# indygreg/python-zstandard

Hardware: NVIDIA H100
Metric: uncompressed GB/s (compress+decompress) (higher is better)
Workload: dtype u8

## Files before the change

python_zstandard_b200/csrc/zb_decode.cu:

```cuda
#include "zb_common.cuh"
#ifdef ZB_SIMT_EMULATION
#define ZB_DYN_SMEM(name) u8* const name = simt_dyn_smem;
#else
#define ZB_DYN_SMEM(name) extern __shared__ __align__(16) u8 name[];
#endif

#ifdef ZB_DEBUG_BLOCKS
#include <cstdio>
#endif

__constant__ u8 c_LL_bits[36] = {0,0,0,0,0,0,0,0,0,0,0,0,0,0,0,0,1,1,1,1,2,2,3,3,4,6,7,8,9,10,11,12,13,14,15,16};
__constant__ u8 c_ML_bits[53] = {0,0,0,0,0,0,0,0,0,0,0,0,0,0,0,0,0,0,0,0,0,0,0,0,0,0,0,0,0,0,0,0,
                                 1,1,1,1,2,2,3,3,4,4,5,7,8,9,10,11,12,13,14,15,16};
__constant__ u32 c_LL_base[36] = {0,1,2,3,4,5,6,7,8,9,10,11,12,13,14,15,16,18,20,22,24,28,32,40,48,64,
                                  0x80,0x100,0x200,0x400,0x800,0x1000,0x2000,0x4000,0x8000,0x10000};
__constant__ u32 c_ML_base[53] = {3,4,5,6,7,8,9,10,11,12,13,14,15,16,17,18,19,20,21,22,23,24,25,26,27,28,29,30,31,32,33,34,
                                  35,37,39,41,43,47,51,59,67,83,99,0x83,0x103,0x203,0x403,0x803,0x1003,0x2003,0x4003,0x8003,0x10003};
__constant__ short c_LL_defnorm[36] = {4,3,2,2,2,2,2,2,2,2,2,2,2,1,1,1,2,2,2,2,2,2,2,2,2,3,2,1,1,1,1,1,-1,-1,-1,-1};
__constant__ short c_ML_defnorm[53] = {1,4,3,2,2,2,2,2,2,1,1,1,1,1,1,1,1,1,1,1,1,1,1,1,1,1,1,1,1,1,1,1,
                                       1,1,1,1,1,1,1,1,1,1,1,1,1,1,-1,-1,-1,-1,-1,-1,-1};
__constant__ short c_OF_defnorm[29] = {1,1,1,1,1,1,2,2,2,1,1,1,1,1,1,1,1,1,1,1,1,1,1,1,-1,-1,-1,-1,-1};

enum { K_LL = 0, K_OF = 1, K_ML = 2 };

// ... 329 lines not shown
        int count; int low = (int)r.peek((u32)(nbits - 1));
        if (low < mx) { count = low; r.skip((u32)(nbits - 1)); }
        else { count = (int)r.peek((u32)nbits); if (count >= threshold) count -= mx; r.skip((u32)nbits); }
        count--;
        remaining -= count < 0 ? -count : count;
        norm[sym++] = (short)count;
        prev0 = !count;
        if (remaining < threshold) {
            if (remaining <= 1) break;
            nbits = zb_hibit((u32)remaining) + 1; threshold = 1 << (nbits - 1);
        }
        if (sym >= max_sv1) break;
    }
    if (remaining != 1 || sym > max_sv1 || r.bp > 8 * n) return 0;
    max_sym = sym - 1;
    return (r.bp + 7) >> 3;
}

__device__ __forceinline__ u32 zb_code_add_bits(u32 sym, int kind)
{
    return kind == K_LL ? c_LL_bits[sym] : (kind == K_ML ? c_ML_bits[sym] : sym);
}

template <typename Cell = ZbFseCell>
__device__ static void zb_build_fse(Cell* t, short* norm, u32 max_sym, u32 log, int kind)
{
    u32 const size = 1u << log, mask = size - 1, step = (size >> 1) + (size >> 3) + 3;
    u32 high = size - 1;
    for (u32 s = 0; s <= max_sym; s++) if (norm[s] == -1) { t[high--] = (Cell)s; norm[s] = 0x4001; }
    u32 pos = 0;
    for (u32 s = 0; s <= max_sym; s++) {
        int const c = norm[s];
        if (c & 0x4000) { norm[s] = 1; continue; }
        for (int i = 0; i < c; i++) { t[pos] = (Cell)s; do pos = (pos + step) & mask; while (pos > high); }
    }
    for (u32 u = 0; u < size; u++) {
        u32 const s = t[u], x = (u32)(u16)norm[s]; norm[s] = (short)(x + 1);
        u32 const nb = log - (u32)zb_hibit(x);
        if constexpr (sizeof(Cell) == 4) t[u] = ZB_CELL((x << nb) - size, nb, zb_code_add_bits(s, kind), s);
        else t[u] = ZB_CELL16(s, x);
    }
}

__global__ void zb_build_default_tables()
{
    if (threadIdx.x == 0 && blockIdx.x == 0) {
        short norm[64];
        for (int i = 0; i < 36; i++) norm[i] = c_LL_defnorm[i];
        zb_build_fse(g_defLL, norm, 35, 6, K_LL);
        for (int i = 0; i < 29; i++) norm[i] = c_OF_defnorm[i];
        zb_build_fse(g_defOF, norm, 28, 5, K_OF);
        for (int i = 0; i < 53; i++) norm[i] = c_ML_defnorm[i];
        zb_build_fse(g_defML, norm, 52, 6, K_ML);
    }
}

struct ZbTab { u32 off; u32 log; };

// ... 1054 lines not shown
                          u32* __restrict__ first_error)
{
    u32 f = blockIdx.x * blockDim.x + threadIdx.x;
    if (f >= n_frames) return;
    ZbSegment s; s.offset = place[f].dst_off; s.length = out_sizes[f];
    out_segs[f] = s;
    if (status[f] != ZB_OK) atomicMin(first_error, f);
}

__global__ void zb_chain_shift(ZbFramePlace* __restrict__ place, u32 n_entries, u64 carry)
{
    u32 const i = blockIdx.x * blockDim.x + threadIdx.x;
    if (i < n_entries) place[i].dst_off += carry;
}

__global__ void zb_digest_dict(const u8* __restrict__ dict, u32 n, ZbDictDigest* __restrict__ out)
{
    if (threadIdx.x || blockIdx.x) return;
    out->status = ZB_OK; out->has_entropy = 0; out->dict_id = 0; out->content_off = 0;
    if (n < 8 || zb_rd32(dict) != ZB_MAGIC_DICT) return;
    out->dict_id = zb_rd32(dict + 4);
    const u8* p = dict + 8; const u8* const end = dict + n;
    {
        __align__(16) u8 ws[256]; u32 rank[13], log, nsym;
#ifdef __CUDA_ARCH__
        __shared__ __align__(16) u8 ring[64];
#else
        u8* const ring = nullptr;
#endif
        u32 const used = zb_huf_weights(ws, p, (u32)(end - p), log, nsym, rank, ring);
        if (!used) { out->status = ZB_E_DICT_CORRUPTED; return; }
        zb_huf_fill(out->huf, ws, log, nsym, rank, 0, 0);
        out->huf_log = log; p += used;
        u32 mxs = 0;
        for (u32 i = 0; i < 256; i++) {
            u32 const wt = i < nsym ? (ws[i >> 1] >> ((i & 1) * 4)) & 15 : 0;
            out->c_huf_nb[i] = wt ? (u8)(log + 1 - wt) : 0; if (wt) mxs = i;
        }
        out->c_huf_max = mxs;
    }
    short norm[64]; u32 mx, log, used;
    mx = 31; used = zb_read_ncount(norm, mx, log, p, (u32)(end - p));
    if (!used || log > 8) { out->status = ZB_E_DICT_CORRUPTED; return; }
    for (u32 i = 0; i < 32; i++) out->c_norm_of[i] = i <= mx ? norm[i] : 0; out->c_max_of = mx;
    zb_build_fse(out->of, norm, mx, log, K_OF); out->of_log = log; p += used;
    mx = 52; used = zb_read_ncount(norm, mx, log, p, (u32)(end - p));
    if (!used || log > 9) { out->status = ZB_E_DICT_CORRUPTED; return; }
// ... 187 lines not shown
```

python_zstandard_b200/csrc/zb_entropy.cuh:

```cuda
#pragma once

#define ZB_ENT_WS_BYTES   256
#define ZB_ENT_DEF_LL     512
#define ZB_ENT_DEF_OF     (ZB_ENT_DEF_LL + 2 * 64)
#define ZB_ENT_DEF_ML     (ZB_ENT_DEF_OF + 2 * 32)
#define ZB_ENT_HEAD_BYTES (ZB_ENT_DEF_ML + 2 * 64)
#define ZB_ENT_POOL_BYTES(W) ((((227 * 1024 - ZB_ENT_HEAD_BYTES) / (W))) & ~15)
#define ZB_ENT_SMEM(W)    ((W) * ZB_ENT_POOL_BYTES(W) + ZB_ENT_HEAD_BYTES)

enum : u32 { ZB_SRC_NONE = 0, ZB_SRC_PREDEF = 1, ZB_SRC_RLE = 2, ZB_SRC_NCOUNT = 3, ZB_SRC_DICT = 4 };
struct ZbTabSrc { u32 kind; u32 sym; const u8* p; u32 n; };

enum : u32 { ZB_BD_FIRST = 1, ZB_BD_FSE_VALID = 2, ZB_BD_SKIP = 4 };
struct ZbBlkDesc {
    u64 hdr_off;
    u64 seq_off, lit_off;
    u32 span;
    u32 frame;
    u32 flags;
    u32 block_max;
    ZbTabSrc dHuf, dLL, dOF, dML;
};
struct ZbBlkExit { u32 rep[3]; u32 err; };

__device__ __forceinline__ u32 zb_warp_incl_scan(u32 v, u32 lane)
{
    #pragma unroll
    for (int d = 1; d < 32; d <<= 1) { u32 y = __shfl_up_sync(0xFFFFFFFFu, v, d); if (lane >= (u32)d) v += y; }
    return v;
}

__device__ static u32 zb_huf_weights(u8* ws, const u8* s, u32 n, u32& out_log, u32& out_nsym, u32* rank, ZB_RING_ARG(ring))
{
    u8* const wn = ws;
    u16* const wt = (u16*)(ws + 128);
    u32 nsym, hdr;
    if (n == 0) return 0;
    #pragma unroll
    for (int i = 0; i < 13; i++) rank[i] = 0;
    for (int i = 0; i < 32; i++) ((u32*)wn)[i] = 0;
    u32 total = 0;
    auto put = [&](u32 i, u32 w) { wn[i >> 1] |= (u8)(w << ((i & 1) * 4)); };
    if (s[0] >= 128) {
        nsym = (u32)s[0] - 127; hdr = (nsym + 1) / 2;
        if (hdr + 1 > n) return 0;
        for (u32 i = 0; i < nsym; i++) {
            u32 b = s[1 + i / 2], w = (i & 1) ? (b & 15) : (b >> 4);
            if (w > 12) return 0;
            put(i, w); rank[w]++; total += (1u << w) >> 1;
        }
    } else {
        hdr = s[0];
        if (hdr + 1 > n) return 0;
        short norm[16]; u32 max_sym = 255, log;
        {
            short nn[256];
            u32 used = zb_read_ncount(nn, max_sym, log, s + 1, hdr);
            if (used == 0 || log > 6) return 0;
            for (u32 i = 16; i <= max_sym; i++) if (nn[i]) return 0;
            if (max_sym > 15) max_sym = 15;
            for (u32 i = 0; i <= max_sym; i++) norm[i] = nn[i];
            u32 const size = 1u << log, mask = size - 1, step = (size >> 1) + (size >> 3) + 3;
            u32 high = size - 1, pos = 0;
            u8 next[16];
            for (u32 sy = 0; sy <= max_sym; sy++) {
                if (norm[sy] == -1) { wt[high--] = (u16)sy; next[sy] = 1; } else next[sy] = (u8)norm[sy];
            }
            for (u32 sy = 0; sy <= max_sym; sy++) {
                int const c = norm[sy];
                for (int i = 0; i < c; i++) { wt[pos] = (u16)sy; do pos = (pos + step) & mask; while (pos > high); }
            }
            for (u32 u = 0; u < size; u++) {
                u32 const sy = wt[u], x = next[sy]++;
                u32 const nb = log - (u32)zb_hibit(x);
                wt[u] = (u16)(sy | (nb << 4) | (((x << nb) - size) << 8));
            }
            ZbBitR<4> b;
            if (!b.init(s + 1 + used, hdr - used, ring)) return 0;
            u32 s1 = b.read(log), s2 = b.read(log); b.refill();
            if (b.left() < 0) return 0;
            nsym = 0;
            for (;;) {
                if (nsym + 2 > 255) return 0;
                { u32 c = wt[s1], w = c & 15; if (w > 12) return 0; put(nsym, w); rank[w]++; total += (1u << w) >> 1; nsym++;
                  s1 = (c >> 8) + b.read((c >> 4) & 15); b.refill(); }
                if (b.left() < 0) { u32 w = wt[s2] & 15; if (w > 12) return 0; put(nsym, w); rank[w]++; total += (1u << w) >> 1; nsym++; break; }
                if (nsym + 2 > 255) return 0;
                { u32 c = wt[s2], w = c & 15; if (w > 12) return 0; put(nsym, w); rank[w]++; total += (1u << w) >> 1; nsym++;
                  s2 = (c >> 8) + b.read((c >> 4) & 15); b.refill(); }
                if (b.left() < 0) { u32 w = wt[s1] & 15; if (w > 12) return 0; put(nsym, w); rank[w]++; total += (1u << w) >> 1; nsym++; break; }
            }
        }
    }
    if (total == 0) return 0;
    u32 const log = (u32)zb_hibit(total) + 1;
    if (log > 12) return 0;
    u32 const rest = (1u << log) - total, hb = (u32)zb_hibit(rest);
    if ((1u << hb) != rest) return 0;
    put(nsym, hb + 1); rank[hb + 1]++; nsym++;
    if (rank[1] < 2 || (rank[1] & 1)) return 0;
    out_log = log; out_nsym = nsym;
    return hdr + 1;
}

#define ZB_HUF_COARSE 8u
struct ZbHufTab { const u16* cells; u32 log, shift, T, base; };
__device__ __forceinline__ void zb_huf_shape(u32 log, const u32* rank, u32& shift, u32& T, u32& base, u32& bytes)
{
    shift = log > ZB_HUF_COARSE ? log - ZB_HUF_COARSE : 0u;
    T = 0; for (u32 wt = 1; wt <= shift; wt++) T += rank[wt] << (wt - 1);
    base = (T + 3u) & ~3u;
    bytes = 2u * (base + (1u << (log - shift)));
}
__device__ __forceinline__ ZbHufTab zb_huf_full(const u16* cells, u32 log) { ZbHufTab t; t.cells = cells; t.log = log; t.shift = 0; t.T = 0; t.base = 0; return t; }
#define ZB_HCELL(t, v) ((t).cells[(v) < (t).T ? (v) : (t).base + ((v) >> (t).shift)])

__device__ static void zb_huf_fill(u16* cells, const u8* ws, u32 log, u32 nsym, const u32* rank, u32 shift, u32 base)
{
    u32 start[13]; { u32 p = 0; for (u32 wt = 1; wt <= 12; wt++) { start[wt] = p; p += wt <= log ? (rank[wt] << (wt - 1)) : 0; } }
    for (u32 i = 0; i < nsym; i++) {
        u32 const wt = (ws[i >> 1] >> ((i & 1) * 4)) & 15; if (!wt) continue;
        u32 len = 1u << (wt - 1), p = start[wt]; start[wt] = p + len;
        if (wt > shift) { len >>= shift; p = base + (p >> shift); }
        u32 const cell = i | ((log + 1 - wt) << 8);
        if (len >= 4) { u64 const v = cell * 0x0001000100010001ull; u64* q = (u64*)(cells + p); for (u32 k = 0; k < len / 4; k++) q[k] = v; }
        else if (len == 2) *(u32*)(cells + p) = cell * 0x00010001u;
        else cells[p] = (u16)cell;
    }
}

__device__ static bool zb_huf_stream2(u8* out, u32 n_out, const u8* s, u32 n, ZbHufTab const t, u8* ring)
{
    ZbBitR<4> b;
    if (!b.init(s, n, ring)) return false;
    u32 const log = t.log;
    u32 i = 0;
    while (i < n_out && ((uintptr_t)(out + i) & 3)) { u32 v = b.peek(log); u32 c = ZB_HCELL(t, v); out[i++] = (u8)c; b.skip(c >> 8); b.refill(); }
    for (; i + 4 <= n_out; i += 4) {
        u32 v0 = b.peek(log); u32 c0 = ZB_HCELL(t, v0); b.skip(c0 >> 8);
        u32 v1 = b.peek(log); u32 c1 = ZB_HCELL(t, v1); b.skip(c1 >> 8); b.refill();
        u32 v2 = b.peek(log); u32 c2 = ZB_HCELL(t, v2); b.skip(c2 >> 8);
        u32 v3 = b.peek(log); u32 c3 = ZB_HCELL(t, v3); b.skip(c3 >> 8); b.refill();
        *(u32*)(out + i) = (c0 & 255) | ((c1 & 255) << 8) | ((c2 & 255) << 16) | (c3 << 24);
    }
    for (; i < n_out; i++) { u32 v = b.peek(log); u32 c = ZB_HCELL(t, v); out[i] = (u8)c; b.skip(c >> 8); b.refill(); }
    return b.left() == 0;
}

struct ZbHufLane { ZbBitR<4> b; u8* out; u32 left; };

__device__ __forceinline__ void zb_huf_one(ZbHufLane& h, ZbHufTab const& t)
{
// ... 66 lines not shown
{
    zb_cta_for(1u << log, [&](u32 i) { u32 const c = src[i]; ((u16*)dst)[i] = ZB_CELL16(ZB_CELL_SYM(c), (ZB_CELL_NEXT(c) + (1u << log)) >> ZB_CELL_NB(c)); });
}

template <int W>
__device__ __forceinline__ u32 zb_ent_head(u8* smem, ZbDictDev const& dict)
{
    u32* const lutLL = (u32*)smem; u32* const lutML = lutLL + 36;
    zb_cta_for(36, [&](u32 i) { lutLL[i] = c_LL_base[i] | ((u32)c_LL_bits[i] << 24); });
    zb_cta_for(53, [&](u32 i) { lutML[i] = c_ML_base[i] | ((u32)c_ML_bits[i] << 24); });
    zb_cta_cells16(smem + ZB_ENT_DEF_LL, g_defLL, 6);
    zb_cta_cells16(smem + ZB_ENT_DEF_OF, g_defOF, 5);
    zb_cta_cells16(smem + ZB_ENT_DEF_ML, g_defML, 6);
    u32 head = ZB_ENT_HEAD_BYTES;
    if (dict.has_entropy) {
        zb_cta_cells16(smem + head, dict.ll, dict.ll_log); head += 2u << dict.ll_log;
        zb_cta_cells16(smem + head, dict.of, dict.of_log); head += 2u << dict.of_log;
        zb_cta_cells16(smem + head, dict.ml, dict.ml_log); head += 2u << dict.ml_log;
    }
    __syncthreads();
    return ((ZB_ENT_SMEM(W) - head) / W) & ~15u;
}

template <bool SYMREP>
__device__ __forceinline__ u32 zb_seq_block(const u8* smem, u8* q, u8* ws, ZbDictDev const& dict,
                                            ZbTabSrc const& dLL, ZbTabSrc const& dOF, ZbTabSrc const& dML,
                                            u32 msLL, u32 msOF, u32 msML, u32 logLL, u32 logOF, u32 logML,
                                            const u8* ip, const u8* bend, u32 nseq, ZbSeq* sq, u32 n_lit, u64 room, u64 hist,
                                            u32& rep0, u32& rep1, u32& rep2, u32& lit_used, u32& produced)
{
    const u32* const lutLL = (const u32*)smem; const u32* const lutML = lutLL + 36;
    short* const normLL = (short*)ws; short* const normOF = normLL + 36; short* const normML = normOF + 32;
    u32 const dct_ll = ZB_ENT_HEAD_BYTES, dct_of = dct_ll + (2u << dict.ll_log), dct_ml = dct_of + (2u << dict.of_log);
    ZbTab tLL, tOF, tML;
    auto setup = [&](const ZbTabSrc& d, short* norm, u32 ms, u32 lg, int kind, u32 dct, u32 dlog, u32 def, u32 deflog, ZbTab& t) {
        if (d.kind == ZB_SRC_NCOUNT) { zb_build_fse((u16*)q, norm, ms, lg, kind); t.off = (u32)(q - smem); t.log = lg; q += 2u << lg; }
        else if (d.kind == ZB_SRC_RLE) { *(u16*)q = ZB_CELL16(d.sym, 1u); t.off = (u32)(q - smem); t.log = 0; q += 2; }
        else if (d.kind == ZB_SRC_DICT) { t.off = dct; t.log = dlog; }
        else { t.off = def; t.log = deflog; }
    };
    setup(dLL, normLL, msLL, logLL, K_LL, dct_ll, dict.ll_log, ZB_ENT_DEF_LL, 6, tLL);
    setup(dOF, normOF, msOF, logOF, K_OF, dct_of, dict.of_log, ZB_ENT_DEF_OF, 5, tOF);
    setup(dML, normML, msML, logML, K_ML, dct_ml, dict.ml_log, ZB_ENT_DEF_ML, 6, tML);

    ZbBitR<8> b;
    if (!b.init(ip, (u32)(bend - ip), ws)) return ZB_E_CORRUPTION;
    u32 sLL = b.read(tLL.log); u32 sOF = b.read(tOF.log); b.refill(); u32 sML = b.read(tML.log);
    const u8* const TL = smem + tLL.off; const u8* const TO = smem + tOF.off; const u8* const TM = smem + tML.off;
    u32 const kL = 31 - tLL.log, kO = 31 - tOF.log, kM = 31 - tML.log;
    u32 err = ZB_OK;
    for (u32 i = 0; i < nseq; i++) {
        u32 const cl = *(const u16*)(TL + 2 * sLL), co = *(const u16*)(TO + 2 * sOF), cm = *(const u16*)(TM + 2 * sML);
        b.refill();
        u32 const llc = cl & 63, ofc = co & 63, xl = cl >> 6, xo = co >> 6, xm = cm >> 6;
        u32 const nl = __clz(xl) - kL, nm = __clz(xm) - kM, no = __clz(xo) - kO;
        u32 const eL = lutLL[llc], eM = lutML[cm & 63];
        u32 const llb = eL >> 24, ab = (eM >> 24) + llb;
        u32 const sb = i + 1 < nseq ? nl + nm + no : 0;
        bool const slow = (int)(ofc + ab + sb) > b.avail;
        u32 const ob = b.read(ofc);
        u32 ll = eL & 0xFFFFFFu, ml = eM & 0xFFFFFFu, off;
        if (ofc > 1) {
            off = (1u << ofc) - 3 + ob;
            if (SYMREP && (off & 0x80000000u)) { err = ZB_E_CORRUPTION; break; }
            rep2 = rep1; rep1 = rep0; rep0 = off;
        } else {
// ... 13 lines not shown
        if (slow) b.refill();
        {
            u32 const both = b.read(ab);
            ml += both >> llb; ll += both & ((1u << llb) - 1);
        }
        if (slow) b.refill();
        {
            u32 const v = b.read(sb);
            sLL = (xl << nl) - (1u << tLL.log) + (v >> (nm + no));
            sML = (xm << nm) - (1u << tML.log) + ((v >> no) & ((1u << nm) - 1));
            sOF = (xo << no) - (1u << tOF.log) + (v & ((1u << no) - 1));
        }
        sq[i] = make_uint4(lit_used, produced, ml, off);
        if ((u64)produced + ll + ml > room) { err = ZB_E_DSTSIZE_TOO_SMALL; break; }
        if (ll > n_lit - lit_used) { err = ZB_E_CORRUPTION; break; }
        lit_used += ll; produced += ll;
        if ((u64)off > hist + produced) { err = ZB_E_CORRUPTION; break; }
        produced += ml;
    }
    if (!err && b.left() != 0) err = ZB_E_CORRUPTION;
    return err;
}

#ifdef ZB_PHASE_TIMERS
__device__ unsigned long long g_zb_ent_phase[8];
#define ZB_EMARK(k) do { if (lane == 0) { long long const t_ = clock64(); atomicAdd(&g_zb_ent_phase[k], (unsigned long long)(t_ - t_ph)); t_ph = t_; } } while (0)
#elif defined(ZB_DEBUG_BLOCKS)
#define ZB_EMARK(k) do { if (err && !(t_ph & 1)) { printf("[emark %d] lane %u err %u\n", k, lane, err); t_ph |= 1; } } while (0)
#else
#define ZB_EMARK(k) do { (void)t_ph; } while (0)
#endif

template <int ZB_ENT_WARPS>
__global__ void __launch_bounds__(ZB_ENT_WARPS * 32)
zb_entropy_decode(const u8* __restrict__ src, const ZbSegment* __restrict__ segs, u32 n_frames,
                  const ZbFramePlace* __restrict__ place, const u64* __restrict__ dst_sizes,
                  ZbBlock* __restrict__ blocks, ZbSeq* __restrict__ seqs, u8* __restrict__ lits,
                  u32* __restrict__ work_counter, ZbDictDev dict, u32* status, u64* __restrict__ out_sizes,
                  u32* __restrict__ ck_expect, u32 take)
{
    ZB_DYN_SMEM(zb_smem);
    u32 const lane = threadIdx.x & 31, warp = threadIdx.x >> 5;
    u32 const pool_bytes = zb_ent_head<ZB_ENT_WARPS>(zb_smem, dict);
    u8* const pool = zb_smem + ZB_ENT_SMEM(ZB_ENT_WARPS) - (ZB_ENT_WARPS - warp) * pool_bytes;
    u8* const ws = pool + lane * ZB_ENT_WS_BYTES;
    u8* const tabs = pool + 32 * ZB_ENT_WS_BYTES;
    u32 const TAB_BYTES = pool_bytes - 32 * ZB_ENT_WS_BYTES;

    for (;;) {
        u32 base = 0;
        if (lane == 0) base = atomicAdd(work_counter, take);
        base = __shfl_sync(0xFFFFFFFFu, base, 0);
        if (base >= n_frames) return;
        u32 const f = base + lane;
        bool done = lane >= take || !(f < n_frames) || status[f] != ZB_OK;

        const u8* s = src; u64 n = 0; ZbHdr h; ZbFramePlace pl; u32 err = ZB_OK;
        u64 cap = 0, out_pos = 0, blk_i = 0, seq_i = 0, lit_i = 0, pos = 0; u32 block_max = 0;
        u32 rep0 = 1, rep1 = 4, rep2 = 8;
        ZbTabSrc dHuf = {ZB_SRC_NONE, 0, nullptr, 0}, dLL = dHuf, dOF = dHuf, dML = dHuf;
        bool fse_valid = false;
        if (!done) {
            s = src + segs[f].offset; n = segs[f].length;
            zb_skip_skippable(s, n);
            zb_parse_header(s, n, h);
            pl = place[f]; cap = pl.dst_cap; blk_i = pl.blk_off; seq_i = pl.seq_off; lit_i = pl.lit_off; pos = h.hdr_size;
            block_max = h.window < ZB_BLOCK_MAX ? (u32)h.window : ZB_BLOCK_MAX;
            if (dict.has_entropy) {
                dHuf.kind = dLL.kind = dOF.kind = dML.kind = ZB_SRC_DICT; fse_valid = true;
                rep0 = dict.rep[0]; rep1 = dict.rep[1]; rep2 = dict.rep[2];
// ... 17 lines not shown
                    if (type == 3) { err = ZB_E_CORRUPTION; break; }
                    if (type == ZB_BLK_RLE) {
                        if (pos + 1 > n) { err = ZB_E_SRCSIZE_WRONG; break; }
                        if (bsize > block_max) { err = ZB_E_CORRUPTION; break; }
                        if (bsize > cap - out_pos) { err = ZB_E_DSTSIZE_TOO_SMALL; break; }
                        B.src_pos = (u64)(s + pos - src); B.regen = bsize; B.lit_byte = s[pos]; pos += 1;
                    } else if (type == ZB_BLK_RAW) {
                        if (pos + bsize > n) { err = ZB_E_SRCSIZE_WRONG; break; }
                        if (bsize > block_max) { err = ZB_E_CORRUPTION; break; }
                        if (bsize > cap - out_pos) { err = ZB_E_DSTSIZE_TOO_SMALL; break; }
                        B.src_pos = (u64)(s + pos - src); B.regen = bsize; pos += bsize;
                    } else {
                        if (pos + bsize > n || bsize > block_max) { err = ZB_E_SRCSIZE_WRONG; break; }
                        bs = s + pos; bend = bs + bsize;
                        err = zb_parse_lit_header(bs, bsize, L);
                        if (err) break;
                        if (L.regen > block_max) { err = ZB_E_CORRUPTION; break; }
                        B.n_lit = L.regen; comp = true;
                    }
                } while (0);
                if (err) { done = true; comp = false; }
            }
            ZB_EMARK(1);
            bool wantH = false; u32 hlog = 0, hns = 0; u32 rank[13]; const u8* hp = nullptr; u32 hleft = 0;
            if (comp) {
                do {
                    if (L.type == 0) {
                        if (L.hdr + L.regen > bsize) { err = ZB_E_CORRUPTION; break; }
                        B.lit_kind = ZB_LIT_RAW; B.src_pos = (u64)(bs + L.hdr - src); ip = bs + L.hdr + L.regen;
                    } else if (L.type == 1) {
                        if (L.hdr + 1 > bsize) { err = ZB_E_CORRUPTION; break; }
                        B.lit_kind = ZB_LIT_RLE; B.lit_byte = bs[L.hdr]; ip = bs + L.hdr + 1;
                    } else {
                        if (L.type == 3 && dHuf.kind == ZB_SRC_NONE) { err = ZB_E_DICT_CORRUPTED; break; }
                        if (!L.single && L.regen < 6) { err = ZB_E_LITERALS_HEADER_WRONG; break; }
                        if (L.csize + L.hdr > bsize || L.regen == 0) { err = ZB_E_CORRUPTION; break; }
                        hp = bs + L.hdr; hleft = L.csize;
                        if (L.type == 2) { dHuf.kind = ZB_SRC_NCOUNT; dHuf.p = hp; dHuf.n = hleft; }
                        if (dHuf.kind == ZB_SRC_NCOUNT) {
                            u32 const used = zb_huf_weights(ws, dHuf.p, dHuf.n, hlog, hns, rank, tabs + lane * 64);
                            if (used == 0 || (L.type == 2 && used >= hleft)) { err = ZB_E_CORRUPTION; break; }
                            if (L.type == 2) { hp += used; hleft -= used; dHuf.n = used; }
                            wantH = true;
                        }
                        B.lit_kind = ZB_LIT_SCRATCH; B.src_pos = lit_i; ip = bs + L.hdr + L.csize;
                    }
                } while (0);
                if (err) { done = true; comp = false; wantH = false; }
            }
            if (comp && B.lit_kind == ZB_LIT_SCRATCH && dHuf.kind == ZB_SRC_DICT) {
                if (!zb_huf_block(lits + lit_i, L.regen, hp, hleft, L.single, zb_huf_full(dict.huf, dict.huf_log), ws)) { err = ZB_E_CORRUPTION; done = true; comp = false; }
            }
            ZB_EMARK(2);
            {
                bool pending = wantH;
                u32 hshift = 0, hT = 0, hbase = 0, hbytes = 0;
                if (wantH) zb_huf_shape(hlog, rank, hshift, hT, hbase, hbytes);
                while (__any_sync(0xFFFFFFFFu, pending)) {
                    u32 const need = pending ? hbytes : 0;
                    u32 const incl = zb_warp_incl_scan((need + 15) & ~15u, lane);
                    if (pending && incl <= TAB_BYTES) {
                        u16* cells = (u16*)(tabs + incl - ((need + 15) & ~15u));
                        zb_huf_fill(cells, ws, hlog, hns, rank, hshift, hbase);
                        ZbHufTab t; t.cells = cells; t.log = hlog; t.shift = hshift; t.T = hT; t.base = hbase;
                        if (!zb_huf_block(lits + lit_i, L.regen, hp, hleft, L.single, t, ws)) { err = ZB_E_CORRUPTION; done = true; comp = false; }
                        pending = false;
                    }
                    __syncwarp();
                }
            }
            ZB_EMARK(3);
            if (comp && B.lit_kind == ZB_LIT_SCRATCH) lit_i += (L.regen + 15) & ~15u;
            u32 nseq = 0, logLL = 0, logOF = 0, logML = 0, msLL = 0, msOF = 0, msML = 0, needS = 0;
            short* const normLL = (short*)ws; short* const normOF = normLL + 36; short* const normML = normOF + 32;
            if (comp) {
                do {
                    if (ip >= bend) { err = ZB_E_SRCSIZE_WRONG; break; }
                    nseq = *ip++;
                    if (nseq > 0x7F) {
                        if (nseq == 0xFF) { if (ip + 2 > bend) { err = ZB_E_SRCSIZE_WRONG; break; } nseq = zb_rd16(ip) + 0x7F00; ip += 2; }
                        else { if (ip >= bend) { err = ZB_E_SRCSIZE_WRONG; break; } nseq = ((nseq - 0x80) << 8) + *ip++; }
                    }
                    B.n_seq = nseq;
                    if (nseq == 0) { if (ip != bend) err = ZB_E_CORRUPTION; break; }
                    if (ip + 1 > bend) { err = ZB_E_SRCSIZE_WRONG; break; }
                    u32 const modes = *ip++;
                    if (modes & 3) { err = ZB_E_CORRUPTION; break; }
                    u32 nd; int r;
                    r = zb_seq_desc(dLL, modes >> 6, 35, 9, ip, (u32)(bend - ip), fse_valid, normLL, logLL, msLL, nd);
                    if (r < 0) { err = ZB_E_CORRUPTION; break; } ip += r; needS += nd;
                    r = zb_seq_desc(dOF, (modes >> 4) & 3, 31, 8, ip, (u32)(bend - ip), fse_valid, normOF, logOF, msOF, nd);
                    if (r < 0) { err = ZB_E_CORRUPTION; break; } ip += r; needS += nd;
                    r = zb_seq_desc(dML, (modes >> 2) & 3, 52, 9, ip, (u32)(bend - ip), fse_valid, normML, logML, msML, nd);
                    if (r < 0) { err = ZB_E_CORRUPTION; break; } ip += r; needS += nd;
                    fse_valid = true;
                } while (0);
                if (err) { done = true; comp = false; nseq = 0; }
            }
            ZB_EMARK(4);
            u32 lit_used = 0, produced = 0;
            {
                bool pending = comp && nseq > 0;
                while (__any_sync(0xFFFFFFFFu, pending)) {
                    u32 const need = pending ? ((needS + 15) & ~15u) : 0;
                    u32 const incl = zb_warp_incl_scan(need, lane);
                    if (pending && incl <= TAB_BYTES) {
                        err = zb_seq_block<false>(zb_smem, tabs + incl - need, ws, dict, dLL, dOF, dML, msLL, msOF, msML, logLL, logOF, logML,
                                                   ip, bend, nseq, seqs + seq_i, L.regen, cap - out_pos, out_pos + hist_extra,
                                                   rep0, rep1, rep2, lit_used, produced);
                        if (err) { done = true; comp = false; }
                        pending = false;
                    }
                    __syncwarp();
                }
            }
            ZB_EMARK(5);
            if (!done) {
                if (comp) {
                    seqs[seq_i + nseq] = make_uint4(lit_used, produced, 0, 0);
                    seq_i += nseq + 1;
                    u32 const tail = L.regen - lit_used;
                    if ((u64)produced + tail > cap - out_pos) err = ZB_E_DSTSIZE_TOO_SMALL;
                    B.regen = produced + tail;
                    if (!err && B.regen > block_max) err = ZB_E_CORRUPTION;
                    pos += bsize;
                }
                if (!err) {
                    blocks[blk_i++] = B;
                    out_pos += B.regen;
                    if (last) {
                        if (h.content_size != ZB_CONTENT_UNKNOWN && out_pos != h.content_size) err = ZB_E_CORRUPTION;
                        else if (h.checksum && pos + 4 > n) err = ZB_E_CHECKSUM_WRONG;
// ... 65 lines not shown
                    if (type == 3) { err = ZB_E_CORRUPTION; break; }
                    if (type == ZB_BLK_RLE) {
                        if (pos + 1 > n) { err = ZB_E_SRCSIZE_WRONG; break; }
                        if (bsize > block_max) { err = ZB_E_CORRUPTION; break; }
                        if (bsize > cap - out_pos) { err = ZB_E_DSTSIZE_TOO_SMALL; break; }
                        B.src_pos = (u64)(s + pos - src); B.regen = bsize; B.lit_byte = s[pos]; pos += 1;
                    } else if (type == ZB_BLK_RAW) {
                        if (pos + bsize > n) { err = ZB_E_SRCSIZE_WRONG; break; }
                        if (bsize > block_max) { err = ZB_E_CORRUPTION; break; }
                        if (bsize > cap - out_pos) { err = ZB_E_DSTSIZE_TOO_SMALL; break; }
                        B.src_pos = (u64)(s + pos - src); B.regen = bsize; pos += bsize;
                    } else {
                        if (pos + bsize > n || bsize > block_max) { err = ZB_E_SRCSIZE_WRONG; break; }
                        bs = s + pos; bend = bs + bsize;
                        err = zb_parse_lit_header(bs, bsize, L);
                        if (err) break;
                        if (L.regen > block_max) { err = ZB_E_CORRUPTION; break; }
                        B.n_lit = L.regen; comp = true;
                    }
                } while (0);
                if (err) { done = true; comp = false; }
            }
            ZB_EMARK(1);
            bool wantH = false; u32 hlog = 0, hns = 0; u32 rank[13]; const u8* hp = nullptr; u32 hleft = 0;
            if (comp) {
                do {
                    if (L.type == 0) {
                        if (L.hdr + L.regen > bsize) { err = ZB_E_CORRUPTION; break; }
                        B.lit_kind = ZB_LIT_RAW; B.src_pos = (u64)(bs + L.hdr - src); ip = bs + L.hdr + L.regen;
                    } else if (L.type == 1) {
                        if (L.hdr + 1 > bsize) { err = ZB_E_CORRUPTION; break; }
                        B.lit_kind = ZB_LIT_RLE; B.lit_byte = bs[L.hdr]; ip = bs + L.hdr + 1;
                    } else {
                        if (L.type == 3 && dHuf.kind == ZB_SRC_NONE) { err = ZB_E_DICT_CORRUPTED; break; }
                        if (!L.single && L.regen < 6) { err = ZB_E_LITERALS_HEADER_WRONG; break; }
                        if (L.csize + L.hdr > bsize || L.regen == 0) { err = ZB_E_CORRUPTION; break; }
                        hp = bs + L.hdr; hleft = L.csize;
                        if (L.type == 2) { dHuf.kind = ZB_SRC_NCOUNT; dHuf.p = hp; dHuf.n = hleft; }
                        if (dHuf.kind == ZB_SRC_NCOUNT) {
                            u32 const used = zb_huf_weights(ws, dHuf.p, dHuf.n, hlog, hns, rank, tabs + lane * 64);
                            if (used == 0 || (L.type == 2 && used >= hleft)) { err = ZB_E_CORRUPTION; break; }
                            if (L.type == 2) { hp += used; hleft -= used; dHuf.n = used; }
                            wantH = true;
                        }
                        B.lit_kind = ZB_LIT_SCRATCH; B.src_pos = lit_i; ip = bs + L.hdr + L.csize;
                    }
                } while (0);
                if (err) { done = true; comp = false; wantH = false; }
            }
            if (comp && B.lit_kind == ZB_LIT_SCRATCH && dHuf.kind == ZB_SRC_DICT) {
                if (!zb_huf_block(lits + lit_i, L.regen, hp, hleft, L.single, zb_huf_full(dict.huf, dict.huf_log), ws)) { err = ZB_E_CORRUPTION; done = true; comp = false; }
            }
            ZB_EMARK(2);
            {
                bool pending = wantH;
                u32 hshift = 0, hT = 0, hbase = 0, hbytes = 0;
                if (wantH) zb_huf_shape(hlog, rank, hshift, hT, hbase, hbytes);
                while (__any_sync(0xFFFFFFFFu, pending)) {
                    u32 const need = pending ? hbytes : 0;
                    u32 const incl = zb_warp_incl_scan((need + 15) & ~15u, lane);
                    if (pending && incl <= TAB_BYTES) {
                        u16* cells = (u16*)(tabs + incl - ((need + 15) & ~15u));
                        zb_huf_fill(cells, ws, hlog, hns, rank, hshift, hbase);
                        ZbHufTab t; t.cells = cells; t.log = hlog; t.shift = hshift; t.T = hT; t.base = hbase;
                        if (!zb_huf_block(lits + lit_i, L.regen, hp, hleft, L.single, t, ws)) { err = ZB_E_CORRUPTION; done = true; comp = false; }
                        pending = false;
                    }
                    __syncwarp();
                }
            }
            ZB_EMARK(3);
            if (comp && B.lit_kind == ZB_LIT_SCRATCH) lit_i += (L.regen + 15) & ~15u;
            u32 nseq = 0, logLL = 0, logOF = 0, logML = 0, msLL = 0, msOF = 0, msML = 0, needS = 0;
            short* const normLL = (short*)ws; short* const normOF = normLL + 36; short* const normML = normOF + 32;
            if (comp) {
                do {
                    if (ip >= bend) { err = ZB_E_SRCSIZE_WRONG; break; }
                    nseq = *ip++;
                    if (nseq > 0x7F) {
                        if (nseq == 0xFF) { if (ip + 2 > bend) { err = ZB_E_SRCSIZE_WRONG; break; } nseq = zb_rd16(ip) + 0x7F00; ip += 2; }
                        else { if (ip >= bend) { err = ZB_E_SRCSIZE_WRONG; break; } nseq = ((nseq - 0x80) << 8) + *ip++; }
                    }
                    B.n_seq = nseq;
                    if (nseq == 0) { if (ip != bend) err = ZB_E_CORRUPTION; break; }
                    if (ip + 1 > bend) { err = ZB_E_SRCSIZE_WRONG; break; }
                    u32 const modes = *ip++;
                    if (modes & 3) { err = ZB_E_CORRUPTION; break; }
                    u32 nd; int r;
                    r = zb_seq_desc(dLL, modes >> 6, 35, 9, ip, (u32)(bend - ip), fse_valid, normLL, logLL, msLL, nd);
                    if (r < 0) { err = ZB_E_CORRUPTION; break; } ip += r; needS += nd;
                    r = zb_seq_desc(dOF, (modes >> 4) & 3, 31, 8, ip, (u32)(bend - ip), fse_valid, normOF, logOF, msOF, nd);
                    if (r < 0) { err = ZB_E_CORRUPTION; break; } ip += r; needS += nd;
                    r = zb_seq_desc(dML, (modes >> 2) & 3, 52, 9, ip, (u32)(bend - ip), fse_valid, normML, logML, msML, nd);
                    if (r < 0) { err = ZB_E_CORRUPTION; break; } ip += r; needS += nd;
                    fse_valid = true;
                } while (0);
                if (err) { done = true; comp = false; nseq = 0; }
            }
            ZB_EMARK(4);
            u32 lit_used = 0, produced = 0;
            {
                bool pending = comp && nseq > 0;
                while (__any_sync(0xFFFFFFFFu, pending)) {
                    u32 const need = pending ? ((needS + 15) & ~15u) : 0;
                    u32 const incl = zb_warp_incl_scan(need, lane);
                    if (pending && incl <= TAB_BYTES) {
                        err = zb_seq_block<true>(zb_smem, tabs + incl - need, ws, dict, dLL, dOF, dML, msLL, msOF, msML, logLL, logOF, logML,
                                                   ip, bend, nseq, seqs + seq_i, L.regen, cap - out_pos, out_pos + hist_extra,
                                                   rep0, rep1, rep2, lit_used, produced);
                        if (err) { done = true; comp = false; }
                        pending = false;
                    }
                    __syncwarp();
                }
            }
            ZB_EMARK(5);
            if (!done) {
                if (comp) {
                    seqs[seq_i + nseq] = make_uint4(lit_used, produced, 0, 0);
                    seq_i += nseq + 1;
                    u32 const tail = L.regen - lit_used;
                    if ((u64)produced + tail > cap - out_pos) err = ZB_E_DSTSIZE_TOO_SMALL;
                    B.regen = produced + tail;
                    if (!err && B.regen > block_max) err = ZB_E_CORRUPTION;
                    pos += bsize;
                }
                if (!err) blocks[blk_i] = B;
                done = true;
            }
        }
        if (lane < take && bi < n_blocks && !(D.flags & ZB_BD_SKIP)) {
            ZbBlkExit X; X.rep[0] = rep0; X.rep[1] = rep1; X.rep[2] = rep2; X.err = err;
// ... 11 lines not shown
```

Baseline: 140.9.

## Pack Huffman rank counters into registers and skew per-lane shared workspaces

Replaces the u32 rank[13] and start[13] arrays with bit-packed register structs whose accesses are fully unrolled selects. This is meant to stop local-memory spills from dynamically indexed arrays. The FSE-to-Huffman weight decode now reuses the shared spread routine with norm stored in the workspace instead of a 256-entry short array on the stack. Per-lane workspace stride and sequence-table allocations get a 16-byte skew to reduce shared-memory bank conflicts, which shrinks the table pool slightly, and phase-timer marks are added.

```diff
diff --git a/python_zstandard_b200/csrc/zb_decode.cu b/python_zstandard_b200/csrc/zb_decode.cu
--- a/python_zstandard_b200/csrc/zb_decode.cu
+++ b/python_zstandard_b200/csrc/zb_decode.cu
@@ -375,8 +375,8 @@
     return kind == K_LL ? c_LL_bits[sym] : (kind == K_ML ? c_ML_bits[sym] : sym);
 }
 
-template <typename Cell = ZbFseCell>
-__device__ static void zb_build_fse(Cell* t, short* norm, u32 max_sym, u32 log, int kind)
+template <typename Cell>
+__device__ __forceinline__ void zb_fse_spread(Cell* t, short* norm, u32 max_sym, u32 log)
 {
     u32 const size = 1u << log, mask = size - 1, step = (size >> 1) + (size >> 3) + 3;
     u32 high = size - 1;
@@ -387,6 +387,13 @@
         if (c & 0x4000) { norm[s] = 1; continue; }
         for (int i = 0; i < c; i++) { t[pos] = (Cell)s; do pos = (pos + step) & mask; while (pos > high); }
     }
+}
+
+template <typename Cell = ZbFseCell>
+__device__ static void zb_build_fse(Cell* t, short* norm, u32 max_sym, u32 log, int kind)
+{
+    zb_fse_spread(t, norm, max_sym, log);
+    u32 const size = 1u << log;
     for (u32 u = 0; u < size; u++) {
         u32 const s = t[u], x = (u32)(u16)norm[s]; norm[s] = (short)(x + 1);
         u32 const nb = log - (u32)zb_hibit(x);
@@ -1487,7 +1494,7 @@
     out->dict_id = zb_rd32(dict + 4);
     const u8* p = dict + 8; const u8* const end = dict + n;
     {
-        __align__(16) u8 ws[256]; u32 rank[13], log, nsym;
+        __align__(16) u8 ws[256]; ZbRank rank; u32 log, nsym;
 #ifdef __CUDA_ARCH__
         __shared__ __align__(16) u8 ring[64];
 #else
diff --git a/python_zstandard_b200/csrc/zb_entropy.cuh b/python_zstandard_b200/csrc/zb_entropy.cuh
--- a/python_zstandard_b200/csrc/zb_entropy.cuh
+++ b/python_zstandard_b200/csrc/zb_entropy.cuh
@@ -1,6 +1,8 @@
 #pragma once
 
 #define ZB_ENT_WS_BYTES   256
+#define ZB_ENT_WS_STRIDE  (ZB_ENT_WS_BYTES + 16)
+#define ZB_ENT_SKEW(b)    ((((b) + 15u) & ~15u) | 16u)
 #define ZB_ENT_DEF_LL     512
 #define ZB_ENT_DEF_OF     (ZB_ENT_DEF_LL + 2 * 64)
 #define ZB_ENT_DEF_ML     (ZB_ENT_DEF_OF + 2 * 32)
@@ -30,66 +32,78 @@
     return v;
 }
 
-__device__ static u32 zb_huf_weights(u8* ws, const u8* s, u32 n, u32& out_log, u32& out_nsym, u32* rank, ZB_RING_ARG(ring))
+template <int WORDS, int BITS>
+struct ZbPacked {
+    static constexpr u32 PER = 32 / BITS, MASK = (1u << BITS) - 1;
+    u32 w[WORDS];
+    __device__ __forceinline__ void clear() {
+        #pragma unroll
+        for (int j = 0; j < WORDS; j++) w[j] = 0;
+    }
+    __device__ __forceinline__ u32 get(u32 i) const {
+        u32 const q = i / PER; u32 v = w[0];
+        #pragma unroll
+        for (int j = 1; j < WORDS; j++) v = q == (u32)j ? w[j] : v;
+        return (v >> (BITS * (i - q * PER))) & MASK;
+    }
+    __device__ __forceinline__ void add(u32 i, u32 v) {
+        u32 const q = i / PER, d = v << (BITS * (i - q * PER));
+        #pragma unroll
+        for (int j = 0; j < WORDS; j++) w[j] += q == (u32)j ? d : 0u;
+    }
+};
+struct ZbRank : ZbPacked<4, 10> {
+    __device__ __forceinline__ u32 operator[](u32 wt) const { return get(wt - 1); }
+    __device__ __forceinline__ void count(u32 wt) { if (wt) add(wt - 1, 1); }
+};
+
+__device__ static u32 zb_huf_weights(u8* ws, const u8* s, u32 n, u32& out_log, u32& out_nsym, ZbRank& rank, ZB_RING_ARG(ring))
 {
     u8* const wn = ws;
     u16* const wt = (u16*)(ws + 128);
     u32 nsym, hdr;
     if (n == 0) return 0;
-    #pragma unroll
-    for (int i = 0; i < 13; i++) rank[i] = 0;
-    for (int i = 0; i < 32; i++) ((u32*)wn)[i] = 0;
+    rank.clear();
     u32 total = 0;
     auto put = [&](u32 i, u32 w) { wn[i >> 1] |= (u8)(w << ((i & 1) * 4)); };
+    auto clear_nibbles = [&] { for (int i = 0; i < 32; i++) ((u32*)wn)[i] = 0; };
     if (s[0] >= 128) {
         nsym = (u32)s[0] - 127; hdr = (nsym + 1) / 2;
         if (hdr + 1 > n) return 0;
+        clear_nibbles();
         for (u32 i = 0; i < nsym; i++) {
             u32 b = s[1 + i / 2], w = (i & 1) ? (b & 15) : (b >> 4);
             if (w > 12) return 0;
-            put(i, w); rank[w]++; total += (1u << w) >> 1;
+            put(i, w); rank.count(w); total += (1u << w) >> 1;
         }
     } else {
         hdr = s[0];
         if (hdr + 1 > n) return 0;
-        short norm[16]; u32 max_sym = 255, log;
-        {
-            short nn[256];
-            u32 used = zb_read_ncount(nn, max_sym, log, s + 1, hdr);
-            if (used == 0 || log > 6) return 0;
-            for (u32 i = 16; i <= max_sym; i++) if (nn[i]) return 0;
-            if (max_sym > 15) max_sym = 15;
-            for (u32 i = 0; i <= max_sym; i++) norm[i] = nn[i];
-            u32 const size = 1u << log, mask = size - 1, step = (size >> 1) + (size >> 3) + 3;
-            u32 high = size - 1, pos = 0;
-            u8 next[16];
-            for (u32 sy = 0; sy <= max_sym; sy++) {
-                if (norm[sy] == -1) { wt[high--] = (u16)sy; next[sy] = 1; } else next[sy] = (u8)norm[sy];
-            }
-            for (u32 sy = 0; sy <= max_sym; sy++) {
-                int const c = norm[sy];
-                for (int i = 0; i < c; i++) { wt[pos] = (u16)sy; do pos = (pos + step) & mask; while (pos > high); }
-            }
-            for (u32 u = 0; u < size; u++) {
-                u32 const sy = wt[u], x = next[sy]++;
-                u32 const nb = log - (u32)zb_hibit(x);
-                wt[u] = (u16)(sy | (nb << 4) | (((x << nb) - size) << 8));
-            }
-            ZbBitR<4> b;
-            if (!b.init(s + 1 + used, hdr - used, ring)) return 0;
-            u32 s1 = b.read(log), s2 = b.read(log); b.refill();
-            if (b.left() < 0) return 0;
-            nsym = 0;
-            for (;;) {
-                if (nsym + 2 > 255) return 0;
-                { u32 c = wt[s1], w = c & 15; if (w > 12) return 0; put(nsym, w); rank[w]++; total += (1u << w) >> 1; nsym++;
-                  s1 = (c >> 8) + b.read((c >> 4) & 15); b.refill(); }
-                if (b.left() < 0) { u32 w = wt[s2] & 15; if (w > 12) return 0; put(nsym, w); rank[w]++; total += (1u << w) >> 1; nsym++; break; }
-                if (nsym + 2 > 255) return 0;
-                { u32 c = wt[s2], w = c & 15; if (w > 12) return 0; put(nsym, w); rank[w]++; total += (1u << w) >> 1; nsym++;
-                  s2 = (c >> 8) + b.read((c >> 4) & 15); b.refill(); }
-                if (b.left() < 0) { u32 w = wt[s1] & 15; if (w > 12) return 0; put(nsym, w); rank[w]++; total += (1u << w) >> 1; nsym++; break; }
-            }
+        short* const norm = (short*)wn; u32 max_sym = 15, log;
+        u32 const used = zb_read_ncount(norm, max_sym, log, s + 1, hdr);
+        if (used == 0 || log > 6) return 0;
+        zb_fse_spread(wt, norm, max_sym, log);
+        u32 const size = 1u << log;
+        for (u32 u = 0; u < size; u++) {
+            u32 const sy = wt[u], x = (u32)(u16)norm[sy]; norm[sy] = (short)(x + 1);
+            u32 const nb = log - (u32)zb_hibit(x);
+            wt[u] = (u16)(sy | (nb << 4) | (((x << nb) - size) << 8));
+        }
+        clear_nibbles();
+        ZbBitR<4> b;
+        if (!b.init(s + 1 + used, hdr - used, ring)) return 0;
+        u32 s1 = b.read(log), s2 = b.read(log); b.refill();
+        if (b.left() < 0) return 0;
+        nsym = 0;
+        for (;;) {
+            if (nsym + 2 > 255) return 0;
+            { u32 c = wt[s1], w = c & 15; if (w > 12) return 0; put(nsym, w); rank.count(w); total += (1u << w) >> 1; nsym++;
+              s1 = (c >> 8) + b.read((c >> 4) & 15); b.refill(); }
+            if (b.left() < 0) { u32 w = wt[s2] & 15; if (w > 12) return 0; put(nsym, w); rank.count(w); total += (1u << w) >> 1; nsym++; break; }
+            if (nsym + 2 > 255) return 0;
+            { u32 c = wt[s2], w = c & 15; if (w > 12) return 0; put(nsym, w); rank.count(w); total += (1u << w) >> 1; nsym++;
+              s2 = (c >> 8) + b.read((c >> 4) & 15); b.refill(); }
+            if (b.left() < 0) { u32 w = wt[s1] & 15; if (w > 12) return 0; put(nsym, w); rank.count(w); total += (1u << w) >> 1; nsym++; break; }
         }
     }
     if (total == 0) return 0;
@@ -97,7 +111,7 @@
     if (log > 12) return 0;
     u32 const rest = (1u << log) - total, hb = (u32)zb_hibit(rest);
     if ((1u << hb) != rest) return 0;
-    put(nsym, hb + 1); rank[hb + 1]++; nsym++;
+    put(nsym, hb + 1); rank.count(hb + 1); nsym++;
     if (rank[1] < 2 || (rank[1] & 1)) return 0;
     out_log = log; out_nsym = nsym;
     return hdr + 1;
@@ -105,22 +119,29 @@
 
 #define ZB_HUF_COARSE 8u
 struct ZbHufTab { const u16* cells; u32 log, shift, T, base; };
-__device__ __forceinline__ void zb_huf_shape(u32 log, const u32* rank, u32& shift, u32& T, u32& base, u32& bytes)
+__device__ __forceinline__ void zb_huf_shape(u32 log, ZbRank const& rank, u32& shift, u32& T, u32& base, u32& bytes)
 {
     shift = log > ZB_HUF_COARSE ? log - ZB_HUF_COARSE : 0u;
-    T = 0; for (u32 wt = 1; wt <= shift; wt++) T += rank[wt] << (wt - 1);
+    T = 0;
+    #pragma unroll
+    for (u32 wt = 1; wt <= 12 - ZB_HUF_COARSE; wt++) T += wt <= shift ? rank[wt] << (wt - 1) : 0u;
     base = (T + 3u) & ~3u;
     bytes = 2u * (base + (1u << (log - shift)));
 }
 __device__ __forceinline__ ZbHufTab zb_huf_full(const u16* cells, u32 log) { ZbHufTab t; t.cells = cells; t.log = log; t.shift = 0; t.T = 0; t.base = 0; return t; }
 #define ZB_HCELL(t, v) ((t).cells[(v) < (t).T ? (v) : (t).base + ((v) >> (t).shift)])
 
-__device__ static void zb_huf_fill(u16* cells, const u8* ws, u32 log, u32 nsym, const u32* rank, u32 shift, u32 base)
-{
-    u32 start[13]; { u32 p = 0; for (u32 wt = 1; wt <= 12; wt++) { start[wt] = p; p += wt <= log ? (rank[wt] << (wt - 1)) : 0; } }
+__device__ static void zb_huf_fill(u16* cells, const u8* ws, u32 log, u32 nsym, ZbRank const& rank, u32 shift, u32 base)
+{
+    ZbPacked<6, 16> next; next.clear();
+    {
+        u32 p = 0;
+        #pragma unroll
+        for (u32 wt = 1; wt <= 12; wt++) { next.add(wt - 1, p); p += wt <= log ? (rank[wt] << (wt - 1)) : 0; }
+    }
     for (u32 i = 0; i < nsym; i++) {
         u32 const wt = (ws[i >> 1] >> ((i & 1) * 4)) & 15; if (!wt) continue;
-        u32 len = 1u << (wt - 1), p = start[wt]; start[wt] = p + len;
+        u32 len = 1u << (wt - 1), p = next.get(wt - 1); next.add(wt - 1, len);
         if (wt > shift) { len >>= shift; p = base + (p >> shift); }
         u32 const cell = i | ((log + 1 - wt) << 8);
         if (len >= 4) { u64 const v = cell * 0x0001000100010001ull; u64* q = (u64*)(cells + p); for (u32 k = 0; k < len / 4; k++) q[k] = v; }
@@ -128,6 +149,25 @@
         else cells[p] = (u16)cell;
     }
 }
+
+#ifdef ZB_SIMT_EMULATION
+__device__ __forceinline__ ZbRank zb_rank_pack(const u32* rank) { ZbRank r; r.clear(); for (u32 wt = 1; wt <= 12; wt++) r.add(wt - 1, rank[wt]); return r; }
+__device__ static u32 zb_huf_weights(u8* ws, const u8* s, u32 n, u32& out_log, u32& out_nsym, u32* rank, ZB_RING_ARG(ring))
+{
+    ZbRank r; u32 const used = zb_huf_weights(ws, s, n, out_log, out_nsym, r, ring);
+    rank[0] = used ? out_nsym : 0;
+    for (u32 w = 1; w <= 12; w++) { rank[w] = used ? r[w] : 0; rank[0] -= rank[w]; }
+    return used;
+}
+__device__ __forceinline__ void zb_huf_shape(u32 log, const u32* rank, u32& shift, u32& T, u32& base, u32& bytes)
+{
+    zb_huf_shape(log, zb_rank_pack(rank), shift, T, base, bytes);
+}
+__device__ static void zb_huf_fill(u16* cells, const u8* ws, u32 log, u32 nsym, const u32* rank, u32 shift, u32 base)
+{
+    zb_huf_fill(cells, ws, log, nsym, zb_rank_pack(rank), shift, base);
+}
+#endif
 
 __device__ static bool zb_huf_stream2(u8* out, u32 n_out, const u8* s, u32 n, ZbHufTab const t, u8* ring)
 {
@@ -240,12 +280,21 @@
     return ((ZB_ENT_SMEM(W) - head) / W) & ~15u;
 }
 
+#ifdef ZB_PHASE_TIMERS
+__device__ unsigned long long g_zb_ent_phase[8];
+#define ZB_EMARK(k) do { if (lane == 0) { long long const t_ = clock64(); atomicAdd(&g_zb_ent_phase[k], (unsigned long long)(t_ - t_ph)); t_ph = t_; } } while (0)
+#elif defined(ZB_DEBUG_BLOCKS)
+#define ZB_EMARK(k) do { if (err && !(t_ph & 1)) { printf("[emark %d] lane %u err %u\n", k, lane, err); t_ph |= 1; } } while (0)
+#else
+#define ZB_EMARK(k) do { (void)t_ph; } while (0)
+#endif
+
 template <bool SYMREP>
 __device__ __forceinline__ u32 zb_seq_block(const u8* smem, u8* q, u8* ws, ZbDictDev const& dict,
                                             ZbTabSrc const& dLL, ZbTabSrc const& dOF, ZbTabSrc const& dML,
                                             u32 msLL, u32 msOF, u32 msML, u32 logLL, u32 logOF, u32 logML,
                                             const u8* ip, const u8* bend, u32 nseq, ZbSeq* sq, u32 n_lit, u64 room, u64 hist,
-                                            u32& rep0, u32& rep1, u32& rep2, u32& lit_used, u32& produced)
+                                            u32& rep0, u32& rep1, u32& rep2, u32& lit_used, u32& produced, long long& t_ph)
 {
     const u32* const lutLL = (const u32*)smem; const u32* const lutML = lutLL + 36;
     short* const normLL = (short*)ws; short* const normOF = normLL + 36; short* const normML = normOF + 32;
@@ -260,6 +309,9 @@
     setup(dLL, normLL, msLL, logLL, K_LL, dct_ll, dict.ll_log, ZB_ENT_DEF_LL, 6, tLL);
     setup(dOF, normOF, msOF, logOF, K_OF, dct_of, dict.of_log, ZB_ENT_DEF_OF, 5, tOF);
     setup(dML, normML, msML, logML, K_ML, dct_ml, dict.ml_log, ZB_ENT_DEF_ML, 6, tML);
+#ifdef ZB_PHASE_TIMERS
+    { u32 const lane = threadIdx.x & 31; ZB_EMARK(7); }
+#endif
 
     ZbBitR<8> b;
     if (!b.init(ip, (u32)(bend - ip), ws)) return ZB_E_CORRUPTION;
@@ -319,15 +371,6 @@
     return err;
 }
 
-#ifdef ZB_PHASE_TIMERS
-__device__ unsigned long long g_zb_ent_phase[8];
-#define ZB_EMARK(k) do { if (lane == 0) { long long const t_ = clock64(); atomicAdd(&g_zb_ent_phase[k], (unsigned long long)(t_ - t_ph)); t_ph = t_; } } while (0)
-#elif defined(ZB_DEBUG_BLOCKS)
-#define ZB_EMARK(k) do { if (err && !(t_ph & 1)) { printf("[emark %d] lane %u err %u\n", k, lane, err); t_ph |= 1; } } while (0)
-#else
-#define ZB_EMARK(k) do { (void)t_ph; } while (0)
-#endif
-
 template <int ZB_ENT_WARPS>
 __global__ void __launch_bounds__(ZB_ENT_WARPS * 32)
 zb_entropy_decode(const u8* __restrict__ src, const ZbSegment* __restrict__ segs, u32 n_frames,
@@ -340,9 +383,9 @@
     u32 const lane = threadIdx.x & 31, warp = threadIdx.x >> 5;
     u32 const pool_bytes = zb_ent_head<ZB_ENT_WARPS>(zb_smem, dict);
     u8* const pool = zb_smem + ZB_ENT_SMEM(ZB_ENT_WARPS) - (ZB_ENT_WARPS - warp) * pool_bytes;
-    u8* const ws = pool + lane * ZB_ENT_WS_BYTES;
-    u8* const tabs = pool + 32 * ZB_ENT_WS_BYTES;
-    u32 const TAB_BYTES = pool_bytes - 32 * ZB_ENT_WS_BYTES;
+    u8* const ws = pool + lane * ZB_ENT_WS_STRIDE;
+    u8* const tabs = pool + 32 * ZB_ENT_WS_STRIDE;
+    u32 const TAB_BYTES = pool_bytes - 32 * ZB_ENT_WS_STRIDE;
 
     for (;;) {
         u32 base = 0;
@@ -406,7 +449,7 @@
                 if (err) { done = true; comp = false; }
             }
             ZB_EMARK(1);
-            bool wantH = false; u32 hlog = 0, hns = 0; u32 rank[13]; const u8* hp = nullptr; u32 hleft = 0;
+            bool wantH = false; u32 hlog = 0, hns = 0; ZbRank rank; const u8* hp = nullptr; u32 hleft = 0;
             if (comp) {
                 do {
                     if (L.type == 0) {
@@ -422,7 +465,7 @@
                         hp = bs + L.hdr; hleft = L.csize;
                         if (L.type == 2) { dHuf.kind = ZB_SRC_NCOUNT; dHuf.p = hp; dHuf.n = hleft; }
                         if (dHuf.kind == ZB_SRC_NCOUNT) {
-                            u32 const used = zb_huf_weights(ws, dHuf.p, dHuf.n, hlog, hns, rank, tabs + lane * 64);
+                            u32 const used = zb_huf_weights(ws, dHuf.p, dHuf.n, hlog, hns, rank, tabs + lane * 80);
                             if (used == 0 || (L.type == 2 && used >= hleft)) { err = ZB_E_CORRUPTION; break; }
                             if (L.type == 2) { hp += used; hleft -= used; dHuf.n = used; }
                             wantH = true;
@@ -446,6 +489,7 @@
                     if (pending && incl <= TAB_BYTES) {
                         u16* cells = (u16*)(tabs + incl - ((need + 15) & ~15u));
                         zb_huf_fill(cells, ws, hlog, hns, rank, hshift, hbase);
+                        ZB_EMARK(6);
                         ZbHufTab t; t.cells = cells; t.log = hlog; t.shift = hshift; t.T = hT; t.base = hbase;
                         if (!zb_huf_block(lits + lit_i, L.regen, hp, hleft, L.single, t, ws)) { err = ZB_E_CORRUPTION; done = true; comp = false; }
                         pending = false;
@@ -486,12 +530,12 @@
             {
                 bool pending = comp && nseq > 0;
                 while (__any_sync(0xFFFFFFFFu, pending)) {
-                    u32 const need = pending ? ((needS + 15) & ~15u) : 0;
+                    u32 const need = pending ? ZB_ENT_SKEW(needS) : 0;
                     u32 const incl = zb_warp_incl_scan(need, lane);
                     if (pending && incl <= TAB_BYTES) {
                         err = zb_seq_block<false>(zb_smem, tabs + incl - need, ws, dict, dLL, dOF, dML, msLL, msOF, msML, logLL, logOF, logML,
                                                    ip, bend, nseq, seqs + seq_i, L.regen, cap - out_pos, out_pos + hist_extra,
-                                                   rep0, rep1, rep2, lit_used, produced);
+                                                   rep0, rep1, rep2, lit_used, produced, t_ph);
                         if (err) { done = true; comp = false; }
                         pending = false;
                     }
@@ -603,7 +647,7 @@
                 if (err) { done = true; comp = false; }
             }
             ZB_EMARK(1);
-            bool wantH = false; u32 hlog = 0, hns = 0; u32 rank[13]; const u8* hp = nullptr; u32 hleft = 0;
+            bool wantH = false; u32 hlog = 0, hns = 0; ZbRank rank; const u8* hp = nullptr; u32 hleft = 0;
             if (comp) {
                 do {
                     if (L.type == 0) {
@@ -643,6 +687,7 @@
                     if (pending && incl <= TAB_BYTES) {
                         u16* cells = (u16*)(tabs + incl - ((need + 15) & ~15u));
                         zb_huf_fill(cells, ws, hlog, hns, rank, hshift, hbase);
+                        ZB_EMARK(6);
                         ZbHufTab t; t.cells = cells; t.log = hlog; t.shift = hshift; t.T = hT; t.base = hbase;
                         if (!zb_huf_block(lits + lit_i, L.regen, hp, hleft, L.single, t, ws)) { err = ZB_E_CORRUPTION; done = true; comp = false; }
                         pending = false;
@@ -688,7 +733,7 @@
                     if (pending && incl <= TAB_BYTES) {
                         err = zb_seq_block<true>(zb_smem, tabs + incl - need, ws, dict, dLL, dOF, dML, msLL, msOF, msML, logLL, logOF, logML,
                                                    ip, bend, nseq, seqs + seq_i, L.regen, cap - out_pos, out_pos + hist_extra,
-                                                   rep0, rep1, rep2, lit_used, produced);
+                                                   rep0, rep1, rep2, lit_used, produced, t_ph);
                         if (err) { done = true; comp = false; }
                         pending = false;
                     }
```

After: 147.7 (median of 6 runs). 4.8% higher.
